# sangminwoo/Temporal-Span-Proposal-Network-VidVRD

Measured on AMD Instinct MI355X. Metric: tracklet-pairs/sec scored (N=32, T=150, D=2048), higher is better.
Workload: dtype f32

## Files before the change

temporal-span-proposal-network-vidvrd_amd/csrc/tspn_wino63.hip:

```cpp
#include <algorithm>
#include <atomic>
#include <type_traits>

#include "tspn_common.h"
#include "tspn_device.h"

namespace {

using namespace tspn_dev;

constexpr int NW = 4;
constexpr int THREADS = 64 * NW;
constexpr int BM = 128;
constexpr int ST = 32;
constexpr int SWG = 64;
constexpr int KC = 8;
constexpr int NJ = 8;
constexpr int VROW = ST * 4;
constexpr int VCH = 2 * NJ * VROW;
constexpr int VHALF = 4 * VCH;
constexpr int VSS = 2 * VHALF;
constexpr int NVB = 2;
constexpr int NPIECE = 16;
constexpr size_t SMEM_BYTES = sizeof(float) * NVB * VSS;
// ... 28 lines not shown
      case 1: u = -2.0 / 9.0 * (g0 + g1 + g2); break;
      case 2: u = -2.0 / 9.0 * (g0 - g1 + g2); break;
      case 3: u = g0 / 90.0 + g1 / 45.0 + 2.0 * g2 / 45.0; break;
      case 4: u = g0 / 90.0 - g1 / 45.0 + 2.0 * g2 / 45.0; break;
      case 5: u = (32.0 * g0 + 16.0 * g1 + 8.0 * g2) / 45.0; break;
      case 6: u = (32.0 * g0 - 16.0 * g1 + 8.0 * g2) / 45.0; break;
      default: u = g2; break;
    }
    out[o] = (float)u;
  }
}

__device__ __forceinline__ void wino63_load_sextet(const float* __restrict__ x, int64_t b, int q, int T, int Cin,
                                                   int64_t ncols, bool ok, int channel_offset, f32x4 (&d)[8]) {
#pragma unroll
  for (int i = 0; i < 8; ++i) {
    const int t = 6 * q + i - 1;
    int64_t n = b * T + t;
    n = n < 0 ? 0 : (n < ncols ? n : ncols - 1);
    const f32x4 v = *reinterpret_cast<const f32x4*>(x + n * Cin + channel_offset);
    d[i] = (ok && t >= 0 && t < T) ? v : f32x4{0.f, 0.f, 0.f, 0.f};
  }
}
__device__ __forceinline__ void wino63_bt(const f32x4 (&d)[8], f32x4 (&V)[8]) {
  V[0] = d[0] - d[6] + 5.25f * (d[4] - d[2]);
  V[7] = d[7] - d[1] + 5.25f * (d[3] - d[5]);
  {
    const f32x4 t1 = d[2] + d[6] - 4.25f * d[4], t2 = d[1] + d[5] - 4.25f * d[3];
    V[1] = t1 + t2;
    V[2] = t1 - t2;
  }
  {
    const f32x4 t1 = d[6] + 0.25f * d[2] - 1.25f * d[4], t2 = 0.5f * d[1] - 2.5f * d[3] + 2.f * d[5];
    V[3] = t1 + t2;
    V[4] = t1 - t2;
  }
  {
    const f32x4 t1 = d[6] + 4.f * (d[2] - 1.25f * d[4]), t2 = 2.f * d[1] - 2.5f * d[3] + 0.5f * d[5];
    V[5] = t1 + t2;
    V[6] = t1 - t2;
  }
}
__device__ __forceinline__ void wino63_absmax_own_frames(const f32x4 (&d)[8], float& m) {
#pragma unroll
  for (int i = 1; i < 7; ++i)
    m = __builtin_elementwise_maximum(
        __builtin_elementwise_maximum(m, __builtin_elementwise_maximum(fabsf(d[i][0]), fabsf(d[i][1]))),
        __builtin_elementwise_maximum(fabsf(d[i][2]), fabsf(d[i][3])));
}
__device__ __forceinline__ void wino63_hot_publish(unsigned long long* __restrict__ hot, unsigned long long key, unsigned slot) {
  key = tspn::wave_max_u64(key);
  if ((threadIdx.x & 63) == 0)
    __hip_atomic_fetch_max(hot + 32 * (slot & (TSPN_CONV_CHECK_HOT_SLOTS - 1)), key, __ATOMIC_RELAXED,
                           __HIP_MEMORY_SCOPE_AGENT);
}

__global__ __launch_bounds__(256) void wino63_input_transform_kernel(
    const float* __restrict__ x, float* __restrict__ Vg, int T, int Cin, int nq, int64_t nsext, int64_t nsp,
    int64_t ncols, unsigned long long* __restrict__ hot) {
  const int lane = threadIdx.x & 63, wave = threadIdx.x >> 6;
  const int cgl = lane & 7, ql = lane >> 3;
  const int64_t S = ((int64_t)blockIdx.x * 4 + wave) * 8 + ql;
  const int cg = blockIdx.y * 8 + cgl;
  if (4 * cg >= Cin) return;
  const bool ok = S < nsext;
  const int64_t b = ok ? S / nq : 0;
  const int q = ok ? (int)(S - b * nq) : 0;
  f32x4 d[8], V[8];
  wino63_load_sextet(x, b, q, T, Cin, ncols, ok, 4 * cg, d);
  if (hot) {
    float m = 0.f;
    wino63_absmax_own_frames(d, m);
    wino63_hot_publish(hot, ((unsigned long long)__float_as_uint(m) << 32) | (unsigned)(S < nsext ? S : 0),
                       blockIdx.x * 4 + wave + 7 * blockIdx.y);
  }
  wino63_bt(d, V);
#pragma unroll
  for (int j = 0; j < 8; ++j)
    *reinterpret_cast<f32x4*>(Vg + (((int64_t)cg * NJ + j) * nsp + S) * 4) = V[j];
}

template <bool BUFV>
__global__ __launch_bounds__(THREADS) __attribute__((amdgpu_waves_per_eu(1, 1))) void conv3_wino63_kernel(
    const float* __restrict__ Vg, const float* __restrict__ Wf, const float* __restrict__ bias,
    float* __restrict__ y, int Cin, int T, int M, int nq, int64_t nsext, int64_t nsp, int tiles_m,
    int tiles_n, int relu, int ldy, int GM, int vec2) {
  extern __shared__ __attribute__((aligned(16))) char smem_raw[];
  float* Vs = reinterpret_cast<float*>(smem_raw);

  int tile_m, tile_n;
  grouped_tile(xcd_remap(blockIdx.x, gridDim.x), GM, tiles_m, tiles_n, tile_m, tile_n);
  const int m0 = tile_m * BM;
  const int64_t S0 = (int64_t)tile_n * SWG;

  const int tid = threadIdx.x;
  const int lane = tid & 63;
  const int wave = __builtin_amdgcn_readfirstlane(tid >> 6);
  const int li = lane & 31, kh = lane >> 5;
  const int nsuper = Cin >> 5;

  const char* abase;
  const unsigned aoff = lane * 16;
  {
    int mb = (m0 >> 5) + wave;
    mb = mb < (M >> 5) ? mb : 0;
    abase = reinterpret_cast<const char*>(Wf) + (int64_t)mb * (Cin / KC) * (NJ * 64 * 16);
  }

  const float* vsrc[BUFV ? 1 : NPIECE];
  unsigned voff[BUFV ? NPIECE : 1];
#pragma unroll
  for (int k = 0; k < NPIECE; ++k) {
    const int pp = NPIECE * wave + k;
    const int rr = 2 * (pp & 31) + kh;
    const int cl = rr >> 4, rem = rr & 15;
    const int g = rem >> 3, j = rem & 7;
    const int64_t e = (((int64_t)(2 * cl + g) * NJ + j) * nsp + S0 + ST * (pp >> 5) + li) * 4;
    if constexpr (BUFV) voff[k] = (unsigned)(e * 4); else vsrc[k] = Vg + e;
  }
  const int64_t super_step = (int64_t)8 * NJ * nsp * 4;
  const __amdgpu_buffer_rsrc_t rsrc_v = buffer_rsrc(Vg, (int)0xffffffffu);
  const unsigned super_bytes = (unsigned)(super_step * 4);
  auto stage_piece = [&](int S, int k) {
    if constexpr (BUFV) {
      const int soff = (int)((unsigned)S * super_bytes);
      bglds16(rsrc_v, voff[k], soff, Vs + (S & 1) * VSS + (NPIECE * wave + k) * 256);
    } else {
      glds16<TSPN_WINO63_VAUX>(vsrc[k], Vs + (S & 1) * VSS + (NPIECE * wave + k) * 256);
    }
    if constexpr (!BUFV) vsrc[k] += super_step;
  };

  f32x16 acc[2][NJ];
#pragma unroll
  for (int cb = 0; cb < 2; ++cb)
#pragma unroll
    for (int j = 0; j < NJ; ++j)
#pragma unroll
      for (int e = 0; e < 16; ++e) acc[cb][j][e] = 0.f;

  f32x4 a[2][NJ], v[2][NJ];
  const float* vlane = Vs + (kh * NJ * ST + li) * 4;
  auto load_v = [&](const float* vbuf, int cl, int j) {
    v[0][j] = *reinterpret_cast<const f32x4*>(vbuf + cl * VCH + j * VROW);
    v[1][j] = *reinterpret_cast<const f32x4*>(vbuf + VHALF + cl * VCH + j * VROW);
  };
  auto load_a_pair = [&](f32x4* ap, auto jp_tag, const char* base) {
    constexpr int JP = decltype(jp_tag)::value;
    if (JP == 0) { load_wfrag<0>(ap[0], aoff, base); load_wfrag<1024>(ap[1], aoff, base); }
    if (JP == 1) { load_wfrag<2048>(ap[2], aoff, base); load_wfrag<3072>(ap[3], aoff, base); }
    if (JP == 2) { load_wfrag<0>(ap[4], aoff, base + 4096); load_wfrag<1024>(ap[5], aoff, base + 4096); }
    if (JP == 3) { load_wfrag<2048>(ap[6], aoff, base + 4096); load_wfrag<3072>(ap[7], aoff, base + 4096); }
  };
  using P0 = std::integral_constant<int, 0>;
  using P1 = std::integral_constant<int, 1>;
  using P2 = std::integral_constant<int, 2>;
  using P3 = std::integral_constant<int, 3>;
  auto mfma_pair = [&](const f32x4* ap, int ja, int jb, int S1, int slot) {
#pragma unroll
    for (int e = 0; e < 4; ++e) {
      acc[0][ja] = __builtin_amdgcn_mfma_f32_32x32x2f32(ap[ja][e], v[0][ja][e], acc[0][ja], 0, 0, 0);
      acc[0][jb] = __builtin_amdgcn_mfma_f32_32x32x2f32(ap[jb][e], v[0][jb][e], acc[0][jb], 0, 0, 0);
      acc[1][ja] = __builtin_amdgcn_mfma_f32_32x32x2f32(ap[ja][e], v[1][ja][e], acc[1][ja], 0, 0, 0);
      if (S1 >= 0) {
        __builtin_amdgcn_sched_barrier(0);
        stage_piece(S1, 4 * slot + e);
        __builtin_amdgcn_sched_barrier(0);
      }
      acc[1][jb] = __builtin_amdgcn_mfma_f32_32x32x2f32(ap[jb][e], v[1][jb][e], acc[1][jb], 0, 0, 0);
    }
  };

#pragma unroll
  for (int k = 0; k < NPIECE; ++k) stage_piece(0, k);
  asm volatile("s_waitcnt vmcnt(0)" ::: "memory");
  __syncthreads();
#pragma unroll
  for (int j = 0; j < NJ; ++j) load_v(vlane, 0, j);
  load_a_pair(a[0], P0{}, abase); load_a_pair(a[0], P1{}, abase); load_a_pair(a[0], P2{}, abase); load_a_pair(a[0], P3{}, abase);
  abase += NJ * 1024;
  load_a_pair(a[1], P0{}, abase); load_a_pair(a[1], P1{}, abase); load_a_pair(a[1], P2{}, abase); load_a_pair(a[1], P3{}, abase);
  abase += NJ * 1024;
  __builtin_amdgcn_sched_barrier(0);

  auto chunk_body = [&](auto cl_tag, const float* vcur, const float* vnext, int S, auto has1_tag, auto has2_tag,
                        auto more_tag) {
    constexpr int CL = decltype(cl_tag)::value;
    constexpr bool HAS1 = decltype(has1_tag)::value;
    constexpr bool HAS2 = decltype(has2_tag)::value;
    constexpr bool MORE = decltype(more_tag)::value;
    constexpr int PAR = CL & 1;
    constexpr int N1 = (HAS1 ? 8 : 0) + ((MORE && CL == 1) ? NPIECE : 0);
    constexpr int N2 = (MORE && CL == 2) ? 6 : 2;
    constexpr int N0 = (HAS2 ? 2 : 0) + ((MORE && CL == 0) ? 4 : 0);
    const int S1 = (MORE && CL == 0) ? S + 1 : -1;
    const float* vn = CL == 3 ? vnext : vcur;
    constexpr int NCL = (CL + 1) & 3;
    f32x4* ap = a[PAR];
    wait_w<3 * N2 + N1>(ap[0], ap[1]);
    mfma_pair(ap, 0, 1, S1, 0);
    if (HAS2) load_a_pair(ap, P0{}, abase);
    if (HAS1) { load_v(vn, NCL, 0); load_v(vn, NCL, 1); }
    __builtin_amdgcn_sched_barrier(0);
    wait_w<2 * N2 + N1 + N0>(ap[2], ap[3]);
    mfma_pair(ap, 2, 3, S1, 1);
    if (HAS2) load_a_pair(ap, P1{}, abase);
    if (HAS1) { load_v(vn, NCL, 2); load_v(vn, NCL, 3); }
    __builtin_amdgcn_sched_barrier(0);
    wait_w<N2 + N1 + 2 * N0>(ap[4], ap[5]);
    mfma_pair(ap, 4, 5, S1, 2);
    if (HAS2) load_a_pair(ap, P2{}, abase);
    if (HAS1) { load_v(vn, NCL, 4); load_v(vn, NCL, 5); }
    __builtin_amdgcn_sched_barrier(0);
    wait_w<N1 + 3 * N0>(ap[6], ap[7]);
    mfma_pair(ap, 6, 7, S1, 3);
    if (HAS2) {
      load_a_pair(ap, P3{}, abase);
      abase += NJ * 1024;
    }
    if (HAS1) { load_v(vn, NCL, 6); load_v(vn, NCL, 7); }
    __builtin_amdgcn_sched_barrier(0);
    if (MORE && CL == 2) {
      asm volatile("s_waitcnt lgkmcnt(0)" ::: "memory");
      __builtin_amdgcn_s_barrier();
      __builtin_amdgcn_sched_barrier(0);
    }
  };
  {
    using TT = std::true_type;
    using FF = std::false_type;
    using C0 = std::integral_constant<int, 0>;
    using C1 = std::integral_constant<int, 1>;
    using C2 = std::integral_constant<int, 2>;
    using C3 = std::integral_constant<int, 3>;
    int S = 0;
    for (; S + 1 < nsuper; ++S) {
      const float* vcur = vlane + (S & 1) * VSS;
      const float* vnext = vlane + ((S + 1) & 1) * VSS;
      chunk_body(C0{}, vcur, vnext, S, TT{}, TT{}, TT{});
      chunk_body(C1{}, vcur, vnext, S, TT{}, TT{}, TT{});
      chunk_body(C2{}, vcur, vnext, S, TT{}, TT{}, TT{});
      chunk_body(C3{}, vcur, vnext, S, TT{}, TT{}, TT{});
    }
    const float* vcur = vlane + (S & 1) * VSS;
    chunk_body(C0{}, vcur, vcur, S, TT{}, TT{}, FF{});
    chunk_body(C1{}, vcur, vcur, S, TT{}, TT{}, FF{});
    chunk_body(C2{}, vcur, vcur, S, TT{}, FF{}, FF{});
    chunk_body(C3{}, vcur, vcur, S, FF{}, FF{}, FF{});
  }

#pragma unroll
  for (int cb = 0; cb < 2; ++cb) {
    const int64_t Sx = S0 + ST * cb + li;
    if (Sx < nsext) {
      const int64_t b = Sx / nq;
      const int q = (int)(Sx - b * nq);
      const int t = 6 * q;
      float* ycol = y + (b * M) * (int64_t)ldy + t;
#pragma unroll
      for (int e = 0; e < 16; ++e) {
        const int m = m0 + wave * 32 + (e & 3) + 8 * (e >> 2) + 4 * kh;
        if (m < M) {
          const float p12 = acc[cb][1][e] + acc[cb][2][e], m12 = acc[cb][1][e] - acc[cb][2][e];
          const float p34 = acc[cb][3][e] + acc[cb][4][e], m34 = acc[cb][3][e] - acc[cb][4][e];
          const float p56 = acc[cb][5][e] + acc[cb][6][e], m56 = acc[cb][5][e] - acc[cb][6][e];
          float o[6];
          o[0] = acc[cb][0][e] + p12 + p34 + p56;
          o[1] = m12 + 2.f * m34 + 0.5f * m56;
          o[2] = p12 + 4.f * p34 + 0.25f * p56;
          o[3] = m12 + 8.f * m34 + 0.125f * m56;
          o[4] = p12 + 16.f * p34 + 0.0625f * p56;
          o[5] = m12 + 32.f * m34 + 0.03125f * m56 + acc[cb][7][e];
          if (bias != nullptr) {
            const float bb = bias[m];
#pragma unroll
            for (int i = 0; i < 6; ++i) o[i] += bb;
          }
          if (relu) {
#pragma unroll
            for (int i = 0; i < 6; ++i) o[i] = tspn::relu_f32(o[i]);
          }
          float* dst = ycol + (int64_t)m * ldy;
          if (vec2) {
            *reinterpret_cast<f32x2*>(dst) = f32x2{o[0], o[1]};
            *reinterpret_cast<f32x2*>(dst + 2) = f32x2{o[2], o[3]};
            *reinterpret_cast<f32x2*>(dst + 4) = f32x2{o[4], o[5]};
          } else {
#pragma unroll
            for (int i = 0; i < 6; ++i)
              if (t + i < T) dst[i] = o[i];
          }
        }
      }
    }
  }
}

constexpr int F_BM = 256, F_BN = 256;
constexpr int F_THREADS = 512;
constexpr int F_ST = 4 * 2 * 256 * 16;
constexpr int F_NST = 4;
constexpr size_t F_SMEM = (size_t)F_NST * F_ST;
constexpr size_t F_SMEM_ALL = F_SMEM + 2 * 256 * sizeof(int);
static_assert(TSPN_WINO63_GM > 0 && TSPN_WINO63_GM < 256, "the contraction's GM argument carries the tail split above bit 7");
constexpr size_t F_PARK_PER_TILE = (size_t)7 * F_THREADS * 128 * sizeof(float);

__device__ __forceinline__ int split_exponent(double mx) {
  if (!(mx > 0.0) || !(mx <= 1.7976931348623157e308)) return 0;
  int k;
  (void)frexp(mx, &k);
  return 15 - k;
}

__device__ __forceinline__ double wino63_u(int j, double g0, double g1, double g2) {
  switch (j) {
    case 0: return g0;
    case 1: return -2.0 / 9.0 * (g0 + g1 + g2);
    case 2: return -2.0 / 9.0 * (g0 - g1 + g2);
    case 3: return g0 / 90.0 + g1 / 45.0 + 2.0 * g2 / 45.0;
    case 4: return g0 / 90.0 - g1 / 45.0 + 2.0 * g2 / 45.0;
    case 5: return (32.0 * g0 + 16.0 * g1 + 8.0 * g2) / 45.0;
    case 6: return (32.0 * g0 - 16.0 * g1 + 8.0 * g2) / 45.0;
    default: return g2;
  }
}

__global__ void pack_wino63_frag_kernel(const float* __restrict__ W, int64_t M, int64_t Cin, int64_t split,
                                        int16_t* __restrict__ out) {
  const int64_t Mp = split ? 2 * M : M, Cp = split ? split : Cin;
  const int64_t ncg = Cp / 8;
  const int64_t o = blockIdx.x * (int64_t)blockDim.x + threadIdx.x;
  if (o >= NJ * Mp) return;
  const int j = (int)(o / Mp);
  const int64_t m = o - j * Mp;
  const float* g = (split && m >= M) ? W + ((m - M) * Cin + split) * 3 : W + (m * Cin) * 3;
  double mx = 0.0;
  for (int64_t c = 0; c < Cp; ++c) {
    const double u = fabs(wino63_u(j, g[3 * c], g[3 * c + 1], g[3 * c + 2]));
    mx = (u > mx || u != u) ? u : mx;
  }
  const int e = split_exponent(mx);
  int16_t* pj = out + (int64_t)j * (2 * ncg + 1) * Mp * 8;
  for (int64_t cg = 0; cg < ncg; ++cg) {
    f16x8 hi, lo;
#pragma unroll
    for (int i = 0; i < 8; ++i) {
      const int64_t c = 8 * cg + i;
      const double u = ldexp(wino63_u(j, g[3 * c], g[3 * c + 1], g[3 * c + 2]), e);
      const _Float16 h = (_Float16)(float)u;
      hi[i] = h;
      lo[i] = (_Float16)(float)(u - (double)(float)h);
    }
    *reinterpret_cast<f16x8*>(pj + (cg * Mp + m) * 8) = hi;
    *reinterpret_cast<f16x8*>(pj + ((ncg + cg) * Mp + m) * 8) = lo;
  }
  *reinterpret_cast<int4*>(pj + (2 * ncg * Mp + m) * 8) = int4{e, 0, 0, 0};
}

__global__ __launch_bounds__(256) void wino63_input_transform_kernel(
    const float* __restrict__ x, _Float16* __restrict__ Vh, int* __restrict__ Ve, int T, int Cin, int nq,
    int64_t nsext, int64_t nsp2, int64_t ncols, unsigned long long* __restrict__ hot) {
  __shared__ float red[4][8][NJ];
  const int tid = threadIdx.x, lane = tid & 63, wave = tid >> 6;
  const int s = tid & 7, cgs = tid >> 3;
  const int64_t S = (int64_t)blockIdx.x * 8 + s;
  const bool ok = S < nsext;
  const int64_t b = ok ? S / nq : 0;
  const int q = ok ? (int)(S - b * nq) : 0;
  const int ncg = Cin >> 3;
  auto transform = [&](int cg, f32x4 (&V)[2][8], bool want_max, float& xmax) {
#pragma unroll
    for (int h = 0; h < 2; ++h) {
      f32x4 d[8];
      wino63_load_sextet(x, b, q, T, Cin, ncols, ok, 8 * cg + 4 * h, d);
      if (want_max) wino63_absmax_own_frames(d, xmax);
      wino63_bt(d, V[h]);
    }
  };
  float cmax[NJ];
#pragma unroll
  for (int j = 0; j < NJ; ++j) cmax[j] = 0.f;
  float xm = 0.f;
  for (int cg = cgs; cg < ncg; cg += 32) {
    f32x4 V[2][8];
    transform(cg, V, hot != nullptr, xm);
#pragma unroll
    for (int j = 0; j < NJ; ++j)
#pragma unroll
      for (int h = 0; h < 2; ++h)
        cmax[j] = __builtin_elementwise_maximum(
            __builtin_elementwise_maximum(cmax[j], __builtin_elementwise_maximum(fabsf(V[h][j][0]), fabsf(V[h][j][1]))),
            __builtin_elementwise_maximum(fabsf(V[h][j][2]), fabsf(V[h][j][3])));
  }
  if (hot)
    wino63_hot_publish(hot, ((unsigned long long)__float_as_uint(xm) << 32) | (unsigned)(ok ? S : 0),
                       blockIdx.x * 4 + wave);
#pragma unroll
  for (int j = 0; j < NJ; ++j) {
    float m = cmax[j];
#pragma unroll
    for (int o = 8; o < 64; o <<= 1) m = __builtin_elementwise_maximum(m, __shfl_xor(m, o, 64));
    if (lane < 8) red[wave][lane][j] = m;
  }
  __syncthreads();
  int ecol[NJ];
#pragma unroll
  for (int j = 0; j < NJ; ++j) {
    const float m = __builtin_elementwise_maximum(__builtin_elementwise_maximum(red[0][s][j], red[1][s][j]),
                                                  __builtin_elementwise_maximum(red[2][s][j], red[3][s][j]));
    ecol[j] = split_exponent((double)m);
  }
  if (cgs == 0) {
#pragma unroll
    for (int j = 0; j < NJ; ++j) Ve[(int64_t)j * nsp2 + S] = ecol[j];
  }
  for (int cg = cgs; cg < ncg; cg += 32) {
    f32x4 V[2][8];
    transform(cg, V, false, xm);
#pragma unroll
    for (int j = 0; j < NJ; ++j) {
      f16x8 hi, lo;
#pragma unroll
      for (int i = 0; i < 8; ++i) {
        const float u = ldexpf(V[i >> 2][j][i & 3], ecol[j]);
        const _Float16 h = (_Float16)u;
        hi[i] = h;
        lo[i] = (_Float16)(u - (float)h);
      }
      _Float16* dst = Vh + (((int64_t)j * 2 * ncg + cg) * nsp2 + S) * 8;
      *reinterpret_cast<f16x8*>(dst) = hi;
      *reinterpret_cast<f16x8*>(dst + (int64_t)ncg * nsp2 * 8) = lo;
    }
  }
}

template <int WN>
__device__ __forceinline__ void wino63_f16x3_tile(
    char* smem_raw, const _Float16* __restrict__ Vh, const int* __restrict__ Ve, const int16_t* __restrict__ Wp,
    const float* __restrict__ bias, float* __restrict__ y, float* __restrict__ park, int Cin, int T, int M, int nq,
    int64_t nsext, int64_t nsp2, int tile_m, int tile_n, int tiles_n, int sub, int relu, int ldy, int vec2) {
  constexpr int MI = WN;
  constexpr int BN = 64 * WN;
  constexpr int NP = 16 + 4 * WN;
  constexpr int PW = (NP + 7) / 8;
  constexpr bool EVEN = NP % 8 == 0;
  const int m0 = tile_m * F_BM;
  const int64_t S0 = (int64_t)tile_n * F_BN + sub * BN;

  const int tid = threadIdx.x;
  const int lane = tid & 63;
  const int wave = __builtin_amdgcn_readfirstlane(tid >> 6);
  const int wm = wave / WN, wn = wave % WN;
  const int li = lane & 31, kh = lane >> 5;
  const int ncg = Cin >> 3, nk = Cin >> 4;
  const int G = NJ * nk;

  const int p0 = wave * NP / 8;
  const int npw = EVEN ? PW : (wave + 1) * NP / 8 - p0;
  const int16_t* src[PW];
  int64_t kstride[PW], jstride[PW];
  int ldst[PW];
#pragma unroll
  for (int i = 0; i < PW; ++i) {
    const int p = min(p0 + i, NP - 1);
    if (p < 16) {
      const int region = p >> 3, cgi = (p >> 2) & 1, r = 64 * (p & 3) + lane;
      src[i] = Wp + (((int64_t)region * ncg + cgi) * M + m0 + r) * 8;
      kstride[i] = (int64_t)2 * M * 8;
      jstride[i] = (int64_t)(2 * ncg + 1) * M * 8;
      ldst[i] = p * 1024;
    } else {
      const int v = p - 16;
      const int region = v / (2 * WN), cgi = (v / WN) & 1, r = 64 * (v % WN) + lane;
      src[i] = reinterpret_cast<const int16_t*>(Vh) + (((int64_t)region * ncg + cgi) * nsp2 + S0 + r) * 8;
      kstride[i] = (int64_t)2 * nsp2 * 8;
      jstride[i] = (int64_t)2 * ncg * nsp2 * 8;
      ldst[i] = (2 + region) * 8192 + cgi * 4096 + (v % WN) * 1024;
    }
  }
  auto issue = [&](int g) {
    const int j = g / nk, k = g - j * nk;
    char* dst = smem_raw + (g & 3) * F_ST;
#pragma unroll
    for (int i = 0; i < PW; ++i)
      if (EVEN || i < npw) glds16(src[i] + j * jstride[i] + k * kstride[i], dst + ldst[i]);
  };
  auto wait_stages = [&](auto ahead_tag) {
    constexpr int AHEAD = decltype(ahead_tag)::value;
    if (EVEN || npw == PW) wait_vmcnt<AHEAD * PW>(); else wait_vmcnt<AHEAD * (PW - 1)>();
  };

  f32x16 acc[MI][2];
#pragma unroll
  for (int mi = 0; mi < MI; ++mi)
#pragma unroll
    for (int ni = 0; ni < 2; ++ni)
#pragma unroll
      for (int e = 0; e < 16; ++e) acc[mi][ni][e] = 0.f;

  float* my_park = park + (int64_t)(tile_m * tiles_n + tile_n) * (F_PARK_PER_TILE / sizeof(float)) +
                   (int64_t)sub * (8 * MI) * F_THREADS * 4 + tid * 4;
  int* etab = reinterpret_cast<int*>(smem_raw + F_SMEM);
  auto unscale = [&](int j) {
    if (tid < F_BM)
      etab[tid] = reinterpret_cast<const int*>(Wp + (int64_t)j * (2 * ncg + 1) * M * 8 + (int64_t)2 * ncg * M * 8)[(int64_t)(m0 + tid) * 4];
    else if (tid - F_BM < BN)
      etab[tid] = Ve[(int64_t)j * nsp2 + S0 + tid - F_BM];
    __syncthreads();
    int ec[2];
#pragma unroll
    for (int ni = 0; ni < 2; ++ni) ec[ni] = etab[F_BM + wn * 64 + ni * 32 + li];
#pragma unroll
    for (int mi = 0; mi < MI; ++mi)
#pragma unroll
      for (int e = 0; e < 16; ++e) {
        const int r = etab[wm * (32 * MI) + mi * 32 + (e & 3) + 8 * (e >> 2) + 4 * kh];
#pragma unroll
        for (int ni = 0; ni < 2; ++ni) acc[mi][ni][e] = ldexpf(acc[mi][ni][e], -(r + ec[ni]));
      }
  };

  issue(0);
  if (G > 1) issue(1);
  if (G > 2) issue(2);
  for (int g = 0; g < G; ++g) {
    if (g + 2 < G) wait_stages(std::integral_constant<int, 2>{});
    else if (g + 1 < G) wait_stages(std::integral_constant<int, 1>{});
    else wait_vmcnt<0>();
    __builtin_amdgcn_sched_barrier(0);
    __builtin_amdgcn_s_barrier();
    __builtin_amdgcn_sched_barrier(0);
    if (g + 3 < G) issue(g + 3);
    __builtin_amdgcn_sched_barrier(0);
    const char* st = smem_raw + (g & 3) * F_ST;
    f16x8 ah[MI], al[MI], bh[2], bl[2];
#pragma unroll
    for (int mi = 0; mi < MI; ++mi) {
      const int off = (kh * 256 + wm * (32 * MI) + mi * 32 + li) * 16;
      ah[mi] = *reinterpret_cast<const f16x8*>(st + off);
      al[mi] = *reinterpret_cast<const f16x8*>(st + 8192 + off);
    }
#pragma unroll
    for (int ni = 0; ni < 2; ++ni) {
      const int off = (kh * 256 + wn * 64 + ni * 32 + li) * 16;
      bh[ni] = *reinterpret_cast<const f16x8*>(st + 16384 + off);
      bl[ni] = *reinterpret_cast<const f16x8*>(st + 24576 + off);
    }
#pragma unroll
    for (int ni = 0; ni < 2; ++ni)
#pragma unroll
      for (int mi = 0; mi < MI; ++mi) acc[mi][ni] = __builtin_amdgcn_mfma_f32_32x32x16_f16(ah[mi], bh[ni], acc[mi][ni], 0, 0, 0);
#pragma unroll
    for (int ni = 0; ni < 2; ++ni)
#pragma unroll
      for (int mi = 0; mi < MI; ++mi) acc[mi][ni] = __builtin_amdgcn_mfma_f32_32x32x16_f16(ah[mi], bl[ni], acc[mi][ni], 0, 0, 0);
#pragma unroll
    for (int ni = 0; ni < 2; ++ni)
#pragma unroll
      for (int mi = 0; mi < MI; ++mi) acc[mi][ni] = __builtin_amdgcn_mfma_f32_32x32x16_f16(al[mi], bh[ni], acc[mi][ni], 0, 0, 0);
    __builtin_amdgcn_sched_barrier(0);
    if (g % nk == nk - 1) {
      const int j = g / nk;
      unscale(j);
      if (j < NJ - 1) {
#pragma unroll
        for (int mi = 0; mi < MI; ++mi)
#pragma unroll
          for (int ni = 0; ni < 2; ++ni)
#pragma unroll
            for (int eq = 0; eq < 4; ++eq) {
              const f32x4 v = {acc[mi][ni][4 * eq], acc[mi][ni][4 * eq + 1], acc[mi][ni][4 * eq + 2], acc[mi][ni][4 * eq + 3]};
              *reinterpret_cast<f32x4*>(my_park + ((int64_t)j * 32 + (mi * 2 + ni) * 4 + eq) * F_THREADS * 4) = v;
#pragma unroll
              for (int e = 0; e < 4; ++e) acc[mi][ni][4 * eq + e] = 0.f;
            }
      }
      __builtin_amdgcn_sched_barrier(0);
    }
  }

  wait_vmcnt<0>();
#pragma unroll
  for (int ni = 0; ni < 2; ++ni) {
    const int64_t Sx = S0 + wn * 64 + ni * 32 + li;
    const bool col_ok = Sx < nsext;
    const int64_t b = col_ok ? Sx / nq : 0;
    const int q = col_ok ? (int)(Sx - b * nq) : 0;
    const int t = 6 * q;
    float* ycol = y + (b * M) * (int64_t)ldy + t;
#pragma unroll
    for (int mi = 0; mi < MI; ++mi)
#pragma unroll
      for (int eq = 0; eq < 4; ++eq) {
        f32x4 P[NJ - 1];
#pragma unroll
        for (int j = 0; j < NJ - 1; ++j)
          P[j] = *reinterpret_cast<const f32x4*>(my_park + ((int64_t)j * 32 + (mi * 2 + ni) * 4 + eq) * F_THREADS * 4);
        if (!col_ok) continue;
#pragma unroll
        for (int e4 = 0; e4 < 4; ++e4) {
          const int e = 4 * eq + e4;
          const int m = m0 + wm * (32 * MI) + mi * 32 + (e & 3) + 8 * (e >> 2) + 4 * kh;
          const float p12 = P[1][e4] + P[2][e4], m12 = P[1][e4] - P[2][e4];
          const float p34 = P[3][e4] + P[4][e4], m34 = P[3][e4] - P[4][e4];
          const float p56 = P[5][e4] + P[6][e4], m56 = P[5][e4] - P[6][e4];
          float o[6];
          o[0] = P[0][e4] + p12 + p34 + p56;
          o[1] = m12 + 2.f * m34 + 0.5f * m56;
          o[2] = p12 + 4.f * p34 + 0.25f * p56;
          o[3] = m12 + 8.f * m34 + 0.125f * m56;
          o[4] = p12 + 16.f * p34 + 0.0625f * p56;
          o[5] = m12 + 32.f * m34 + 0.03125f * m56 + acc[mi][ni][e];
          if (bias != nullptr) {
            const float bb = bias[m];
#pragma unroll
            for (int i = 0; i < 6; ++i) o[i] += bb;
          }
          if (relu) {
#pragma unroll
            for (int i = 0; i < 6; ++i) o[i] = tspn::relu_f32(o[i]);
          }
          float* dst = ycol + (int64_t)m * ldy;
          if (vec2) {
            *reinterpret_cast<f32x2*>(dst) = f32x2{o[0], o[1]};
            *reinterpret_cast<f32x2*>(dst + 2) = f32x2{o[2], o[3]};
            *reinterpret_cast<f32x2*>(dst + 4) = f32x2{o[4], o[5]};
          } else {
#pragma unroll
            for (int i = 0; i < 6; ++i)
              if (t + i < T) dst[i] = o[i];
          }
        }
      }
  }
}

__global__ __launch_bounds__(F_THREADS, 1) void conv3_wino63_kernel(
    const _Float16* __restrict__ Vh, const int* __restrict__ Ve, const int16_t* __restrict__ Wp,
    const float* __restrict__ bias, float* __restrict__ y, float* __restrict__ park, int Cin, int T, int M, int nq,
    int64_t nsext, int64_t nsp2, int tiles_m, int tiles_n, int relu, int ldy, int GM, int vec2) {
  extern __shared__ __attribute__((aligned(16))) char smem_raw[];

  const int f = max((GM >> 8) & 0xff, 1);
  GM &= 0xff;
  const int tiles = tiles_m * tiles_n;
  const int nsplit = f > 1 ? ((int)gridDim.x - tiles) / (f - 1) : 0;
  const int nfull = tiles - nsplit;
  const int bid = blockIdx.x;
  int wg, sub = 0;
  if (bid < nfull) {
    wg = xcd_remap(bid, nfull);
  } else {
    const int s = xcd_remap(bid - nfull, nsplit * f);
    wg = nfull + s / f;
    sub = s - (s / f) * f;
  }
  int tile_m, tile_n;
  grouped_tile(wg, GM, tiles_m, tiles_n, tile_m, tile_n);
  if (bid < nfull)
    wino63_f16x3_tile<4>(smem_raw, Vh, Ve, Wp, bias, y, park, Cin, T, M, nq, nsext, nsp2, tile_m, tile_n, tiles_n, 0, relu, ldy, vec2);
  else if (f == 2)
    wino63_f16x3_tile<2>(smem_raw, Vh, Ve, Wp, bias, y, park, Cin, T, M, nq, nsext, nsp2, tile_m, tile_n, tiles_n, sub, relu, ldy, vec2);
  else
    wino63_f16x3_tile<1>(smem_raw, Vh, Ve, Wp, bias, y, park, Cin, T, M, nq, nsext, nsp2, tile_m, tile_n, tiles_n, sub, relu, ldy, vec2);
}

int64_t padded_sextets(int64_t B, int64_t T) { return tspn::ceil_div(B * tspn::ceil_div(T, 6), SWG) * SWG; }
int64_t padded_sextets_f16x3(int64_t B, int64_t T) { return tspn::ceil_div(B * tspn::ceil_div(T, 6), F_BN) * F_BN; }

struct F16x3Layout {
  size_t v, e, park, total;
};
F16x3Layout f16x3_layout(int64_t B, int64_t T, int64_t Cin, int64_t M) {
  F16x3Layout L{};
  const size_t nsp2 = (size_t)padded_sextets_f16x3(B, T);
  L.v = 0;
  L.e = tspn::align_up((size_t)NJ * 2 * Cin * nsp2 * sizeof(_Float16), 256);
  L.park = L.e + tspn::align_up((size_t)NJ * nsp2 * sizeof(int), 256);
  L.total = L.park + (size_t)tspn::ceil_div(M, F_BM) * (nsp2 / F_BN) * F_PARK_PER_TILE;
  return L;
}

int check_common(const char* what, int64_t B, int64_t T, int64_t Cin, int64_t M, int64_t ldy) {
  TSPN_REQUIRE(B >= 0 && Cin > 0 && T > 0 && M > 0 && ldy >= T && ldy < (1 << 24), TSPN_EINVAL,
               "%s: bad sizes B=%lld T=%lld Cin=%lld M=%lld ldy=%lld", what, (long long)B, (long long)T,
               (long long)Cin, (long long)M, (long long)ldy);
  TSPN_REQUIRE(tspn::wino63_supported(Cin, M), TSPN_EUNSUPPORTED,
               "%s: needs Cin %% 32 == 0, M %% 32 == 0 (Cin=%lld M=%lld)", what, (long long)Cin, (long long)M);
  TSPN_REQUIRE(Cin < (1 << 24) && T < (1 << 24) && M < (1 << 24), TSPN_EUNSUPPORTED, "%s: dimension too large", what);
  return TSPN_OK;
}

}

bool tspn::wino63_supported(int64_t Cin, int64_t M) { return Cin > 0 && M > 0 && Cin % 32 == 0 && M % 32 == 0; }

size_t tspn::wino63_workspace_bytes(int64_t B, int64_t T, int64_t Cin) {
  if (B <= 0 || T <= 0 || Cin <= 0) return 0;
  return (size_t)(Cin / 4) * NJ * (size_t)padded_sextets(B, T) * 4 * sizeof(float);
}

extern "C" size_t tspn_conv3_tc_wino63_workspace_bytes(int64_t B, int64_t T, int64_t Cin) {
  return tspn::wino63_workspace_bytes(B, T, Cin);
}

extern "C" int tspn_pack_conv3_wino63_frag_f32(const float* W, int64_t M, int64_t Cin, int64_t split, float* frag,
                                               void* stream) {
  TSPN_REQUIRE(W && frag, TSPN_EINVAL, "tspn_pack_conv3_wino63_frag_f32: null pointer");
  TSPN_REQUIRE(M > 0 && Cin > 0 && split >= 0, TSPN_EINVAL, "tspn_pack_conv3_wino63_frag_f32: bad sizes");
  TSPN_REQUIRE(split == 0 || Cin == 2 * split, TSPN_EINVAL,
               "tspn_pack_conv3_wino63_frag_f32: split=%lld requires Cin == 2*split (Cin=%lld)", (long long)split,
               (long long)Cin);
  const int64_t Mp = split ? 2 * M : M, Cp = split ? split : Cin;
  TSPN_REQUIRE(Cp % KC == 0 && Mp % 32 == 0, TSPN_EUNSUPPORTED,
               "tspn_pack_conv3_wino63_frag_f32: needs (packed) Cin %% 8 == 0 and M %% 32 == 0 (Cin=%lld M=%lld)",
               (long long)Cp, (long long)Mp);
  const int64_t total = NJ * Cp * Mp;
  const int blocks = (int)std::min<int64_t>(tspn::ceil_div(total, 256), 8192);
  hipLaunchKernelGGL(pack_wino63_frag_kernel, dim3(blocks), dim3(256), 0, TSPN_STREAM(stream), W, M, Cin, split, frag);
  return tspn::check_launch("tspn_pack_conv3_wino63_frag_f32");
}

int tspn::wino63_input_transform(const float* x, int64_t B, int64_t T, int64_t Cin, void* workspace,
                                 size_t workspace_bytes, void* stream, uint64_t* hot) {
  const char* what = "tspn_conv3_tc_wino63_f32(input transform)";
  if (int rc = check_common(what, B, T, Cin, 32, T)) return rc;
  if (B == 0) return TSPN_OK;
  TSPN_REQUIRE(x && tspn::aligned16(x), TSPN_EINVAL, "%s: x must be a 16-byte aligned pointer", what);
  const size_t need = tspn::wino63_workspace_bytes(B, T, Cin);
  TSPN_REQUIRE(workspace && workspace_bytes >= need, TSPN_EWORKSPACE, "%s: workspace %zu < %zu bytes", what,
               workspace_bytes, need);
  TSPN_REQUIRE(tspn::aligned16(workspace), TSPN_EINVAL, "%s: workspace must be 16-byte aligned",
               what);
  const int64_t nq = tspn::ceil_div(T, 6);
  const int64_t nsext = B * nq, nsp = padded_sextets(B, T);
  TSPN_REQUIRE(nsp / 32 < (1LL << 31) && Cin / 32 < 65536, TSPN_EUNSUPPORTED, "%s: grid too large", what);
  hipLaunchKernelGGL(wino63_input_transform_kernel, dim3((unsigned)(nsp / 32), (unsigned)(Cin / 32)), dim3(256), 0,
                     TSPN_STREAM(stream), x, static_cast<float*>(workspace), (int)T, (int)Cin, (int)nq, nsext, nsp,
                     B * T, reinterpret_cast<unsigned long long*>(hot));
  return tspn::check_launch(what);
}

static std::atomic<int> g_piece_form{0};

int tspn::wino63_contract(const void* workspace, int64_t B, int64_t T, int64_t Cin, const float* frag, int64_t M,
                          const float* bias, int relu, float* y, int64_t ldy, void* stream) {
  const char* what = "tspn_conv3_tc_wino63_f32";
  if (int rc = check_common(what, B, T, Cin, M, ldy)) return rc;
  if (B == 0) return TSPN_OK;
  TSPN_REQUIRE(workspace && frag && y, TSPN_EINVAL, "%s: null pointer", what);
  TSPN_REQUIRE(tspn::aligned16(frag) && (reinterpret_cast<uintptr_t>(y) & 3) == 0,
               TSPN_EUNSUPPORTED, "%s: frag must be 16-byte aligned", what);
  const int64_t nq = tspn::ceil_div(T, 6);
  const int64_t nsext = B * nq, nsp = padded_sextets(B, T);
  const int64_t tiles_m = tspn::ceil_div(M, BM), tiles_n = nsp / SWG;
  TSPN_REQUIRE(tiles_m * tiles_n < (1LL << 31), TSPN_EUNSUPPORTED, "%s: grid too large", what);
  const int vec2 = (ldy % 2 == 0) && (ldy >= 6 * nq) && ((reinterpret_cast<uintptr_t>(y) & 7) == 0);
#ifndef TSPN_WINO63_BUFV
#define TSPN_WINO63_BUFV 1
#endif
  const bool bufv = TSPN_WINO63_BUFV && tspn::wino63_workspace_bytes(B, T, Cin) < (1ull << 32) &&
                    g_piece_form.load(std::memory_order_relaxed) == 0;
  static tspn::LdsLimit lds[2];
  auto launch = [&](auto kern, tspn::LdsLimit& lim) {
    if (int rc = lim.ensure(reinterpret_cast<const void*>(kern), SMEM_BYTES, what)) return rc;
    hipLaunchKernelGGL(kern, dim3((unsigned)(tiles_m * tiles_n)), dim3(THREADS), SMEM_BYTES, TSPN_STREAM(stream),
                       static_cast<const float*>(workspace), frag, bias, y, (int)Cin, (int)T, (int)M, (int)nq, nsext, nsp,
                       (int)tiles_m, (int)tiles_n, relu, (int)ldy, TSPN_WINO63_GM, vec2);
    return tspn::check_launch(what);
  };
  return bufv ? launch(conv3_wino63_kernel<true>, lds[1]) : launch(conv3_wino63_kernel<false>, lds[0]);
}

int tspn::conv3_tc_wino63(const float* x, int64_t B, int64_t T, int64_t Cin, const float* frag, int64_t M,
                          const float* bias, int relu, float* y, int64_t ldy, void* workspace,
                          size_t workspace_bytes, void* stream) {
  if (int rc = check_common("tspn_conv3_tc_wino63_f32", B, T, Cin, M, ldy)) return rc;
  if (int rc = tspn::wino63_input_transform(x, B, T, Cin, workspace, workspace_bytes, stream)) return rc;
  return tspn::wino63_contract(workspace, B, T, Cin, frag, M, bias, relu, y, ldy, stream);
}

extern "C" int tspn_conv3_tc_wino63_set_piece_form(int form) {
  TSPN_REQUIRE(form == 0 || form == 1, TSPN_EINVAL, "tspn_conv3_tc_wino63_set_piece_form: form must be 0 or 1");
  return g_piece_form.exchange(form, std::memory_order_relaxed);
}

extern "C" int tspn_conv3_tc_wino63_f32(const float* x, int64_t B, int64_t T, int64_t Cin, const float* frag,
                                        int64_t M, const float* bias, int relu, float* y, void* workspace,
                                        size_t workspace_bytes, void* stream) {
  return tspn::conv3_tc_wino63(x, B, T, Cin, frag, M, bias, relu, y, T, workspace, workspace_bytes, stream);
}

bool tspn::wino63_f16x3_supported(int64_t Cin, int64_t M) {
  return Cin > 0 && M > 0 && Cin % 32 == 0 && M % F_BM == 0 && Cin < (1 << 24) && M < (1 << 24);
}

size_t tspn::wino63_f16x3_workspace_bytes(int64_t B, int64_t T, int64_t Cin, int64_t M) {
  if (B <= 0 || T <= 0 || Cin <= 0 || M <= 0) return 0;
  return f16x3_layout(B, T, Cin, M).total;
}

extern "C" size_t tspn_conv3_tc_wino63_f16x3_workspace_bytes(int64_t B, int64_t T, int64_t Cin, int64_t M) {
  return tspn::wino63_f16x3_workspace_bytes(B, T, Cin, M);
}

extern "C" size_t tspn_pack_conv3_wino63_f16x3_elements(int64_t M, int64_t Cin, int64_t split) {
  if (M <= 0 || Cin <= 0 || split < 0 || (split && Cin != 2 * split)) return 0;
  const int64_t Mp = split ? 2 * M : M, Cp = split ? split : Cin;
  return (size_t)NJ * (2 * (Cp / 8) + 1) * Mp * 8;
}

extern "C" int tspn_pack_conv3_wino63_f16x3(const float* W, int64_t M, int64_t Cin, int64_t split, int16_t* packed,
                                            void* stream) {
  const char* what = "tspn_pack_conv3_wino63_f16x3";
  TSPN_REQUIRE(W && packed, TSPN_EINVAL, "%s: null pointer", what);
  TSPN_REQUIRE(M > 0 && Cin > 0 && split >= 0, TSPN_EINVAL, "%s: bad sizes", what);
  TSPN_REQUIRE(split == 0 || Cin == 2 * split, TSPN_EINVAL, "%s: split=%lld requires Cin == 2*split (Cin=%lld)", what,
               (long long)split, (long long)Cin);
  TSPN_REQUIRE(tspn::aligned16(packed), TSPN_EINVAL, "%s: packed must be 16-byte aligned", what);
  const int64_t Mp = split ? 2 * M : M, Cp = split ? split : Cin;
  TSPN_REQUIRE(tspn::wino63_f16x3_supported(Cp, Mp), TSPN_EUNSUPPORTED,
               "%s: needs (packed) Cin %% 32 == 0 and M %% 256 == 0 (Cin=%lld M=%lld)", what, (long long)Cp, (long long)Mp);
  void (*kern)(const float*, int64_t, int64_t, int64_t, int16_t*) = pack_wino63_frag_kernel;
  hipLaunchKernelGGL(kern, dim3((unsigned)tspn::ceil_div(NJ * Mp, 256)), dim3(256), 0, TSPN_STREAM(stream), W, M, Cin,
                     split, packed);
  return tspn::check_launch(what);
}

int tspn::wino63_f16x3_input_transform(const float* x, int64_t B, int64_t T, int64_t Cin, int64_t M, void* workspace,
                                       size_t workspace_bytes, void* stream, uint64_t* hot) {
  const char* what = "tspn_conv3_tc_wino63_f16x3(input transform)";
  if (int rc = check_common(what, B, T, Cin, 32, T)) return rc;
  TSPN_REQUIRE(tspn::wino63_f16x3_supported(Cin, M), TSPN_EUNSUPPORTED,
               "%s: needs Cin %% 32 == 0 and M %% 256 == 0 (Cin=%lld M=%lld)", what, (long long)Cin, (long long)M);
  if (B == 0) return TSPN_OK;
  TSPN_REQUIRE(x && tspn::aligned16(x), TSPN_EINVAL, "%s: x must be a 16-byte aligned pointer", what);
  const F16x3Layout L = f16x3_layout(B, T, Cin, M);
  TSPN_REQUIRE(workspace && workspace_bytes >= L.total, TSPN_EWORKSPACE, "%s: workspace %zu < %zu bytes", what,
               workspace_bytes, L.total);
  TSPN_REQUIRE((reinterpret_cast<uintptr_t>(workspace) & 255) == 0, TSPN_EINVAL, "%s: workspace must be 256-byte aligned",
               what);
  const int64_t nq = tspn::ceil_div(T, 6);
  const int64_t nsext = B * nq, nsp2 = padded_sextets_f16x3(B, T);
  TSPN_REQUIRE(nsp2 / 8 < (1LL << 31), TSPN_EUNSUPPORTED, "%s: grid too large", what);
  char* ws = static_cast<char*>(workspace);
  void (*kern)(const float*, _Float16*, int*, int, int, int, int64_t, int64_t, int64_t, unsigned long long*) =
      wino63_input_transform_kernel;
  hipLaunchKernelGGL(kern, dim3((unsigned)(nsp2 / 8)), dim3(256), 0, TSPN_STREAM(stream), x,
                     reinterpret_cast<_Float16*>(ws + L.v), reinterpret_cast<int*>(ws + L.e), (int)T, (int)Cin, (int)nq,
                     nsext, nsp2, B * T, reinterpret_cast<unsigned long long*>(hot));
  return tspn::check_launch(what);
}

static std::atomic<int> g_tail_split{1};

extern "C" int tspn_conv3_tc_wino63_f16x3_set_tail_split(int on) {
  TSPN_REQUIRE(on == 0 || on == 1, TSPN_EINVAL, "tspn_conv3_tc_wino63_f16x3_set_tail_split: on must be 0 or 1");
  return g_tail_split.exchange(on, std::memory_order_relaxed);
}

static int device_cus() {
  constexpr int kMaxDevices = 64;
  static std::atomic<int> cached[kMaxDevices] = {};
  int dev = -1, cus = 0;
  if (hipGetDevice(&dev) != hipSuccess) return 0;
  const bool tracked = dev >= 0 && dev < kMaxDevices;
  if (tracked && (cus = cached[dev].load(std::memory_order_relaxed)) > 0) return cus;
  if (hipDeviceGetAttribute(&cus, hipDeviceAttributeMultiprocessorCount, dev) != hipSuccess || cus <= 0) return 0;
  if (tracked) cached[dev].store(cus, std::memory_order_relaxed);
  return cus;
}

static int tail_split_factor(int64_t tiles, int cus, int64_t* R) {
  *R = 0;
  if (cus <= 0 || g_tail_split.load(std::memory_order_relaxed) == 0) return 1;
  const int64_t r = tiles % cus;
  if (r == 0) return 1;
  const int64_t f = std::min<int64_t>(4, cus / r);
  if (f < 2) return 1;
  *R = r;
  return f == 3 ? 2 : (int)f;
}

int tspn::wino63_f16x3_contract(void* workspace, size_t workspace_bytes, int64_t B, int64_t T, int64_t Cin,
                                const int16_t* packed, int64_t M, const float* bias, int relu, float* y, int64_t ldy,
                                void* stream) {
  const char* what = "tspn_conv3_tc_wino63_f16x3";
  if (int rc = check_common(what, B, T, Cin, M, ldy)) return rc;
  TSPN_REQUIRE(tspn::wino63_f16x3_supported(Cin, M), TSPN_EUNSUPPORTED,
               "%s: needs Cin %% 32 == 0 and M %% 256 == 0 (Cin=%lld M=%lld)", what, (long long)Cin, (long long)M);
  if (B == 0) return TSPN_OK;
  TSPN_REQUIRE(workspace && packed && y, TSPN_EINVAL, "%s: null pointer", what);
  TSPN_REQUIRE(tspn::aligned16(packed) && (reinterpret_cast<uintptr_t>(y) & 3) == 0,
               TSPN_EUNSUPPORTED, "%s: packed weights must be 16-byte aligned", what);
  const F16x3Layout L = f16x3_layout(B, T, Cin, M);
  TSPN_REQUIRE(workspace_bytes >= L.total, TSPN_EWORKSPACE, "%s: workspace %zu < %zu bytes", what, workspace_bytes,
               L.total);
  const int64_t nq = tspn::ceil_div(T, 6);
  const int64_t nsext = B * nq, nsp2 = padded_sextets_f16x3(B, T);
  const int64_t tiles_m = M / F_BM, tiles_n = nsp2 / F_BN;
  TSPN_REQUIRE(tiles_m * tiles_n < (1LL << 29), TSPN_EUNSUPPORTED, "%s: grid too large", what);
  const int vec2 = (ldy % 2 == 0) && (ldy >= 6 * nq) && ((reinterpret_cast<uintptr_t>(y) & 7) == 0);
  int64_t R = 0;
  const int f = tail_split_factor(tiles_m * tiles_n, device_cus(), &R);
  const int64_t grid = tiles_m * tiles_n + R * (f - 1);
  char* ws = static_cast<char*>(workspace);
  static tspn::LdsLimit lds;
  void (*kern)(const _Float16*, const int*, const int16_t*, const float*, float*, float*, int, int, int, int, int64_t,
               int64_t, int, int, int, int, int, int) = conv3_wino63_kernel;
  if (int rc = lds.ensure(reinterpret_cast<const void*>(kern), F_SMEM_ALL, what)) return rc;
  hipLaunchKernelGGL(kern, dim3((unsigned)grid), dim3(F_THREADS), F_SMEM_ALL, TSPN_STREAM(stream),
                     reinterpret_cast<const _Float16*>(ws + L.v), reinterpret_cast<const int*>(ws + L.e), packed, bias, y,
                     reinterpret_cast<float*>(ws + L.park), (int)Cin, (int)T, (int)M, (int)nq, nsext, nsp2, (int)tiles_m,
                     (int)tiles_n, relu, (int)ldy, TSPN_WINO63_GM | (f << 8), vec2);
  return tspn::check_launch(what);
}

extern "C" int tspn_conv3_tc_wino63_f16x3(const float* x, int64_t B, int64_t T, int64_t Cin, const int16_t* packed,
                                          int64_t M, const float* bias, int relu, float* y, void* workspace,
                                          size_t workspace_bytes, void* stream) {
  const char* what = "tspn_conv3_tc_wino63_f16x3";
  if (int rc = check_common(what, B, T, Cin, M, T)) return rc;
  TSPN_REQUIRE(tspn::wino63_f16x3_supported(Cin, M), TSPN_EUNSUPPORTED,
               "%s: needs Cin %% 32 == 0 and M %% 256 == 0 (Cin=%lld M=%lld)", what, (long long)Cin, (long long)M);
  if (B > 0) {
    TSPN_REQUIRE(workspace && packed && y, TSPN_EINVAL, "%s: null pointer", what);
    TSPN_REQUIRE(tspn::aligned16(packed) && (reinterpret_cast<uintptr_t>(y) & 3) == 0,
                 TSPN_EUNSUPPORTED, "%s: packed weights must be 16-byte aligned", what);
  }
  if (int rc = tspn::wino63_f16x3_input_transform(x, B, T, Cin, M, workspace, workspace_bytes, stream)) return rc;
  return tspn::wino63_f16x3_contract(workspace, workspace_bytes, B, T, Cin, packed, M, bias, relu, y, T, stream);
}
```

Baseline: 1.101 million.

## Software-pipeline f16x3 Winograd contraction with LDS prefetch, staggered issue, buffer loads

Restructures the main MFMA loop of the f16x3 Winograd contraction. Each k-step now interleaves LDS reads of the next stage's hi operands and the current stage's lo operands with MFMA groups, using sched_group_barrier hints. For the full 4-wide tile, half the waves issue their global-to-LDS copies after the first MFMA group and the other half after the second. Load addresses are now incremented pointers instead of being recomputed per step, and when the slab fits in 31 bits and piece form is off, the copies use buffer-resource loads. The aim is to hide LDS and global-load latency behind MFMA work and to cut address arithmetic, at the cost of more register pressure and more complex control flow.

Measured after the change: 1.221 million, median of 6. 1.11x the previous value.

```diff
diff --git a/temporal-span-proposal-network-vidvrd_amd/csrc/tspn_wino63.hip b/temporal-span-proposal-network-vidvrd_amd/csrc/tspn_wino63.hip
--- a/temporal-span-proposal-network-vidvrd_amd/csrc/tspn_wino63.hip
+++ b/temporal-span-proposal-network-vidvrd_amd/csrc/tspn_wino63.hip
@@ -354,7 +354,7 @@
 constexpr int F_NST = 4;
 constexpr size_t F_SMEM = (size_t)F_NST * F_ST;
 constexpr size_t F_SMEM_ALL = F_SMEM + 2 * 256 * sizeof(int);
-static_assert(TSPN_WINO63_GM > 0 && TSPN_WINO63_GM < 256, "the contraction's GM argument carries the tail split above bit 7");
+static_assert(TSPN_WINO63_GM > 0 && TSPN_WINO63_GM < 256, "the contraction's GM argument carries the tail split and the piece form above bit 7");
 constexpr size_t F_PARK_PER_TILE = (size_t)7 * F_THREADS * 128 * sizeof(float);
 
 __device__ __forceinline__ int split_exponent(double mx) {
@@ -486,7 +486,10 @@
   }
 }
 
-template <int WN>
+#ifndef TSPN_WINO63_F16X3_STAGGER
+#define TSPN_WINO63_F16X3_STAGGER 1
+#endif
+template <int WN, bool BUF>
 __device__ __forceinline__ void wino63_f16x3_tile(
     char* smem_raw, const _Float16* __restrict__ Vh, const int* __restrict__ Ve, const int16_t* __restrict__ Wp,
     const float* __restrict__ bias, float* __restrict__ y, float* __restrict__ park, int Cin, int T, int M, int nq,
@@ -496,6 +499,7 @@
   constexpr int NP = 16 + 4 * WN;
   constexpr int PW = (NP + 7) / 8;
   constexpr bool EVEN = NP % 8 == 0;
+  constexpr bool STAGGER = TSPN_WINO63_F16X3_STAGGER && WN == 4;
   const int m0 = tile_m * F_BM;
   const int64_t S0 = (int64_t)tile_n * F_BN + sub * BN;
 
@@ -510,32 +514,48 @@
   const int p0 = wave * NP / 8;
   const int npw = EVEN ? PW : (wave + 1) * NP / 8 - p0;
   const int16_t* src[PW];
-  int64_t kstride[PW], jstride[PW];
+  unsigned voff[PW];
   int ldst[PW];
 #pragma unroll
   for (int i = 0; i < PW; ++i) {
     const int p = min(p0 + i, NP - 1);
+    int64_t el;
     if (p < 16) {
       const int region = p >> 3, cgi = (p >> 2) & 1, r = 64 * (p & 3) + lane;
-      src[i] = Wp + (((int64_t)region * ncg + cgi) * M + m0 + r) * 8;
-      kstride[i] = (int64_t)2 * M * 8;
-      jstride[i] = (int64_t)(2 * ncg + 1) * M * 8;
+      el = (((int64_t)region * ncg + cgi) * M + m0 + r) * 8;
+      src[i] = Wp + el;
       ldst[i] = p * 1024;
     } else {
       const int v = p - 16;
       const int region = v / (2 * WN), cgi = (v / WN) & 1, r = 64 * (v % WN) + lane;
-      src[i] = reinterpret_cast<const int16_t*>(Vh) + (((int64_t)region * ncg + cgi) * nsp2 + S0 + r) * 8;
-      kstride[i] = (int64_t)2 * nsp2 * 8;
-      jstride[i] = (int64_t)2 * ncg * nsp2 * 8;
+      el = (((int64_t)region * ncg + cgi) * nsp2 + S0 + r) * 8;
+      src[i] = reinterpret_cast<const int16_t*>(Vh) + el;
       ldst[i] = (2 + region) * 8192 + cgi * 4096 + (v % WN) * 1024;
     }
-  }
-  auto issue = [&](int g) {
-    const int j = g / nk, k = g - j * nk;
-    char* dst = smem_raw + (g & 3) * F_ST;
+    voff[i] = (unsigned)(el * 2);
+  }
+  int ik = 0, ist = 0;
+  const char* wbase = reinterpret_cast<const char*>(Wp);
+  const char* vbase = reinterpret_cast<const char*>(Vh);
+  auto issue = [&]() {
+    char* dst = smem_raw + ist * F_ST;
 #pragma unroll
     for (int i = 0; i < PW; ++i)
-      if (EVEN || i < npw) glds16(src[i] + j * jstride[i] + k * kstride[i], dst + ldst[i]);
+      if (EVEN || i < npw) {
+        if (BUF) bglds16(buffer_rsrc_unbounded(p0 + i < 16 ? wbase : vbase), voff[i], 0, dst + ldst[i]);
+        else glds16(src[i], dst + ldst[i]);
+      }
+    ist = (ist + 1) & 3;
+    const bool wrap = ++ik == nk;
+    if (wrap) ik = 0;
+    const int64_t dw = (int64_t)M * (wrap ? 32 * nk + 48 : 32), dv = nsp2 * (wrap ? 32 * nk + 32 : 32);
+    if (BUF) {
+      wbase += dw;
+      vbase += dv;
+    } else {
+#pragma unroll
+      for (int i = 0; i < PW; ++i) src[i] = reinterpret_cast<const int16_t*>(reinterpret_cast<const char*>(src[i]) + (p0 + i < 16 ? dw : dv));
+    }
   };
   auto wait_stages = [&](auto ahead_tag) {
     constexpr int AHEAD = decltype(ahead_tag)::value;
@@ -572,64 +592,93 @@
       }
   };
 
-  issue(0);
-  if (G > 1) issue(1);
-  if (G > 2) issue(2);
-  for (int g = 0; g < G; ++g) {
-    if (g + 2 < G) wait_stages(std::integral_constant<int, 2>{});
-    else if (g + 1 < G) wait_stages(std::integral_constant<int, 1>{});
+  f16x8 ah[MI], al[MI], bh[2][2], bl[2];
+  const int a_off = (kh * 256 + wm * (32 * MI) + li) * 16, b_off = (kh * 256 + wn * 64 + li) * 16;
+  auto read_hi = [&](int st, f16x8 (&bhn)[2]) {
+    const char* s = smem_raw + st * F_ST;
+#pragma unroll
+    for (int mi = 0; mi < MI; ++mi) ah[mi] = *reinterpret_cast<const f16x8*>(s + a_off + mi * 512);
+#pragma unroll
+    for (int ni = 0; ni < 2; ++ni) bhn[ni] = *reinterpret_cast<const f16x8*>(s + 16384 + b_off + ni * 512);
+  };
+  auto read_lo = [&](int st) {
+    const char* s = smem_raw + st * F_ST;
+#pragma unroll
+    for (int ni = 0; ni < 2; ++ni) bl[ni] = *reinterpret_cast<const f16x8*>(s + 24576 + b_off + ni * 512);
+#pragma unroll
+    for (int mi = 0; mi < MI; ++mi) al[mi] = *reinterpret_cast<const f16x8*>(s + 8192 + a_off + mi * 512);
+  };
+  auto group = [&](const f16x8 (&a)[MI], const f16x8 (&b)[2]) {
+#pragma unroll
+    for (int ni = 0; ni < 2; ++ni)
+#pragma unroll
+      for (int mi = 0; mi < MI; ++mi) acc[mi][ni] = __builtin_amdgcn_mfma_f32_32x32x16_f16(a[mi], b[ni], acc[mi][ni], 0, 0, 0);
+  };
+  auto point_end = [&](int j) {
+    unscale(j);
+    if (j < NJ - 1) {
+#pragma unroll
+      for (int mi = 0; mi < MI; ++mi)
+#pragma unroll
+        for (int ni = 0; ni < 2; ++ni)
+#pragma unroll
+          for (int eq = 0; eq < 4; ++eq) {
+            const f32x4 v = {acc[mi][ni][4 * eq], acc[mi][ni][4 * eq + 1], acc[mi][ni][4 * eq + 2], acc[mi][ni][4 * eq + 3]};
+            *reinterpret_cast<f32x4*>(my_park + ((int64_t)j * 32 + (mi * 2 + ni) * 4 + eq) * F_THREADS * 4) = v;
+#pragma unroll
+            for (int e = 0; e < 4; ++e) acc[mi][ni][4 * eq + e] = 0.f;
+          }
+    }
+    __builtin_amdgcn_sched_barrier(0);
+  };
+  auto kstep = [&](int g, f16x8 (&bc)[2], f16x8 (&bn)[2], auto steady_tag) {
+    constexpr bool STEADY = decltype(steady_tag)::value;
+#define TSPN_MR(NM, NR)                                \
+  __builtin_amdgcn_sched_group_barrier(0x008, NM, 0);  \
+  __builtin_amdgcn_sched_group_barrier(0x100, NR, 0);
+    group(ah, bc);
+    read_lo(g & 3);
+    if (WN == 4) { TSPN_MR(1, 1) TSPN_MR(1, 1) TSPN_MR(1, 1) TSPN_MR(1, 1) TSPN_MR(1, 1) TSPN_MR(1, 1) TSPN_MR(2, 0) }
+    __builtin_amdgcn_sched_barrier(0);
+    if (STEADY || g + 2 < G) wait_stages(std::integral_constant<int, 1>{});
     else wait_vmcnt<0>();
-    __builtin_amdgcn_sched_barrier(0);
     __builtin_amdgcn_s_barrier();
     __builtin_amdgcn_sched_barrier(0);
-    if (g + 3 < G) issue(g + 3);
+    const bool more = STEADY || g + 3 < G;
+    if (more && (!STAGGER || wm == 0)) issue();
     __builtin_amdgcn_sched_barrier(0);
-    const char* st = smem_raw + (g & 3) * F_ST;
-    f16x8 ah[MI], al[MI], bh[2], bl[2];
-#pragma unroll
-    for (int mi = 0; mi < MI; ++mi) {
-      const int off = (kh * 256 + wm * (32 * MI) + mi * 32 + li) * 16;
-      ah[mi] = *reinterpret_cast<const f16x8*>(st + off);
-      al[mi] = *reinterpret_cast<const f16x8*>(st + 8192 + off);
-    }
-#pragma unroll
-    for (int ni = 0; ni < 2; ++ni) {
-      const int off = (kh * 256 + wn * 64 + ni * 32 + li) * 16;
-      bh[ni] = *reinterpret_cast<const f16x8*>(st + 16384 + off);
-      bl[ni] = *reinterpret_cast<const f16x8*>(st + 24576 + off);
-    }
-#pragma unroll
-    for (int ni = 0; ni < 2; ++ni)
-#pragma unroll
-      for (int mi = 0; mi < MI; ++mi) acc[mi][ni] = __builtin_amdgcn_mfma_f32_32x32x16_f16(ah[mi], bh[ni], acc[mi][ni], 0, 0, 0);
-#pragma unroll
-    for (int ni = 0; ni < 2; ++ni)
-#pragma unroll
-      for (int mi = 0; mi < MI; ++mi) acc[mi][ni] = __builtin_amdgcn_mfma_f32_32x32x16_f16(ah[mi], bl[ni], acc[mi][ni], 0, 0, 0);
-#pragma unroll
-    for (int ni = 0; ni < 2; ++ni)
-#pragma unroll
-      for (int mi = 0; mi < MI; ++mi) acc[mi][ni] = __builtin_amdgcn_mfma_f32_32x32x16_f16(al[mi], bh[ni], acc[mi][ni], 0, 0, 0);
+    group(ah, bl);
     __builtin_amdgcn_sched_barrier(0);
-    if (g % nk == nk - 1) {
-      const int j = g / nk;
-      unscale(j);
-      if (j < NJ - 1) {
-#pragma unroll
-        for (int mi = 0; mi < MI; ++mi)
-#pragma unroll
-          for (int ni = 0; ni < 2; ++ni)
-#pragma unroll
-            for (int eq = 0; eq < 4; ++eq) {
-              const f32x4 v = {acc[mi][ni][4 * eq], acc[mi][ni][4 * eq + 1], acc[mi][ni][4 * eq + 2], acc[mi][ni][4 * eq + 3]};
-              *reinterpret_cast<f32x4*>(my_park + ((int64_t)j * 32 + (mi * 2 + ni) * 4 + eq) * F_THREADS * 4) = v;
-#pragma unroll
-              for (int e = 0; e < 4; ++e) acc[mi][ni][4 * eq + e] = 0.f;
-            }
-      }
-      __builtin_amdgcn_sched_barrier(0);
-    }
-  }
+    if (STAGGER && more && wm != 0) issue();
+    __builtin_amdgcn_sched_barrier(0);
+    group(al, bc);
+    if (STEADY || g + 1 < G) read_hi((g + 1) & 3, bn);
+    if (WN == 4 && STEADY) { TSPN_MR(2, 1) TSPN_MR(1, 1) TSPN_MR(1, 1) TSPN_MR(1, 1) TSPN_MR(1, 1) TSPN_MR(1, 1) TSPN_MR(1, 0) }
+#undef TSPN_MR
+    __builtin_amdgcn_sched_barrier(0);
+  };
+
+  issue();
+  issue();
+  issue();
+  wait_stages(std::integral_constant<int, 2>{});
+  __builtin_amdgcn_s_barrier();
+  __builtin_amdgcn_sched_barrier(0);
+  read_hi(0, bh[0]);
+  int g = 0, kc = 0, jc = 0;
+  auto pair = [&](auto steady_tag) {
+    kstep(g, bh[0], bh[1], steady_tag);
+    kstep(g + 1, bh[1], bh[0], steady_tag);
+    g += 2;
+    kc += 2;
+    if (kc == nk) {
+      point_end(jc);
+      kc = 0;
+      ++jc;
+    }
+  };
+  while (g + 4 < G) pair(std::true_type{});
+  while (g < G) pair(std::false_type{});
 
   wait_vmcnt<0>();
 #pragma unroll
@@ -694,6 +743,7 @@
   extern __shared__ __attribute__((aligned(16))) char smem_raw[];
 
   const int f = max((GM >> 8) & 0xff, 1);
+  const bool buf = (GM >> 16) & 1;
   GM &= 0xff;
   const int tiles = tiles_m * tiles_n;
   const int nsplit = f > 1 ? ((int)gridDim.x - tiles) / (f - 1) : 0;
@@ -709,12 +759,16 @@
   }
   int tile_m, tile_n;
   grouped_tile(wg, GM, tiles_m, tiles_n, tile_m, tile_n);
-  if (bid < nfull)
-    wino63_f16x3_tile<4>(smem_raw, Vh, Ve, Wp, bias, y, park, Cin, T, M, nq, nsext, nsp2, tile_m, tile_n, tiles_n, 0, relu, ldy, vec2);
-  else if (f == 2)
-    wino63_f16x3_tile<2>(smem_raw, Vh, Ve, Wp, bias, y, park, Cin, T, M, nq, nsext, nsp2, tile_m, tile_n, tiles_n, sub, relu, ldy, vec2);
-  else
-    wino63_f16x3_tile<1>(smem_raw, Vh, Ve, Wp, bias, y, park, Cin, T, M, nq, nsext, nsp2, tile_m, tile_n, tiles_n, sub, relu, ldy, vec2);
+  auto tile = [&](auto wn_tag, auto buf_tag) {
+    wino63_f16x3_tile<decltype(wn_tag)::value, decltype(buf_tag)::value>(
+        smem_raw, Vh, Ve, Wp, bias, y, park, Cin, T, M, nq, nsext, nsp2, tile_m, tile_n, tiles_n, sub, relu, ldy, vec2);
+  };
+  auto shape = [&](auto buf_tag) {
+    if (bid < nfull) tile(std::integral_constant<int, 4>{}, buf_tag);
+    else if (f == 2) tile(std::integral_constant<int, 2>{}, buf_tag);
+    else tile(std::integral_constant<int, 1>{}, buf_tag);
+  };
+  if (buf) shape(std::true_type{}); else shape(std::false_type{});
 }
 
 int64_t padded_sextets(int64_t B, int64_t T) { return tspn::ceil_div(B * tspn::ceil_div(T, 6), SWG) * SWG; }
@@ -956,6 +1010,8 @@
   int64_t R = 0;
   const int f = tail_split_factor(tiles_m * tiles_n, device_cus(), &R);
   const int64_t grid = tiles_m * tiles_n + R * (f - 1);
+  const int64_t slab = 4 * Cin * std::max<int64_t>(M, nsp2);
+  const int buf = slab < (1LL << 31) && g_piece_form.load(std::memory_order_relaxed) == 0;
   char* ws = static_cast<char*>(workspace);
   static tspn::LdsLimit lds;
   void (*kern)(const _Float16*, const int*, const int16_t*, const float*, float*, float*, int, int, int, int, int64_t,
@@ -964,7 +1020,7 @@
   hipLaunchKernelGGL(kern, dim3((unsigned)grid), dim3(F_THREADS), F_SMEM_ALL, TSPN_STREAM(stream),
                      reinterpret_cast<const _Float16*>(ws + L.v), reinterpret_cast<const int*>(ws + L.e), packed, bias, y,
                      reinterpret_cast<float*>(ws + L.park), (int)Cin, (int)T, (int)M, (int)nq, nsext, nsp2, (int)tiles_m,
-                     (int)tiles_n, relu, (int)ldy, TSPN_WINO63_GM | (f << 8), vec2);
+                     (int)tiles_n, relu, (int)ldy, TSPN_WINO63_GM | (f << 8) | (buf << 16), vec2);
   return tspn::check_launch(what);
 }
 
```
